# wagnva/semantic-nerf-for-satellite-data

Measured on AMD Instinct MI355X. Metric: train rays/sec (4096 rays x 64 samples), higher is better.
Workload: dtype f32(f16x2)

## Files before the change

### semantic-nerf-for-satellite-data_amd/csrc/api.hip

```cpp
#include <stdarg.h>
#include <stdio.h>
#include <stdlib.h>
#include <string.h>

#include <mutex>

#include "aux_kernels.h"
#include "bsp.h"
#include "composite.h"
#include "gemm.h"
#include "plan.h"

namespace snerf {

int forward_bsp(const Plan& p, const float* pk, const SnerfInputs* in, const SnerfOutputs* out, void* workspace, hipStream_t st);
int backward_bsp(const Plan& p, const float* pk, const SnerfInputs* in, const SnerfOutGrads* go, float* gp, float* d_t, float* d_t_s,
                 void* workspace, hipStream_t st);

static thread_local char g_err[512] = "";
void set_error(const char* fmt, ...) {
  va_list ap;
  va_start(ap, fmt);
  vsnprintf(g_err, sizeof(g_err), fmt, ap);
  va_end(ap);
// ... 195 lines not shown
  size_t off = 0;
  auto take = [&](size_t n) { size_t o = off; off += round_up_sz(n, 64); return o; };
  for (int i = 0; i < p.L; ++i) {
    p.k_tr[i] = (i == 0) ? p.Ep : (((p.skip_mask >> i) & 1u) ? p.Ep + p.W : p.W);
    p.w_tr[i] = take((size_t)p.W * p.k_tr[i]);
    p.b_tr[i] = take(p.W);
  }
  p.w_fs = take((size_t)(p.W + NARROW) * p.W); p.b_fs = take(p.W + NARROW);
  p.w_h1 = take((size_t)p.N1 * p.FA); p.b_h1 = take(p.N1);
  p.w_s2 = take((size_t)p.H * p.H); p.b_s2 = take(p.H);
  p.w_s3 = take((size_t)p.H * p.H); p.b_s3 = take(p.H);
  p.w_s4 = take((size_t)NARROW * p.H); p.b_s4 = take(NARROW);
  p.w_fin = take((size_t)NARROW * p.KF); p.b_fin = take(NARROW);
  p.sky_floats = 9 * p.H + 4;
  p.sky = take(p.sky_floats);
  p.n_fp32 = off;
  {
    const char* ev = getenv("SNERF_COMPOSE_FEATS");
    p.compose_feats = p.pl == 2 && (p.H & 31) == 0 && p.N1 + NARROW <= 2048 && !(ev && ev[0] == '0' && ev[1] == 0);
  }
  if (!p.compose_feats) { plan_weights(p); plan_bsp(p); return SNERF_OK; }
  Plan q = p;
  q.compose_feats = false;
  plan_weights(q);
  plan_bsp(q);
  plan_weights(p);
  plan_bsp(p);
  if (q.packed_floats > p.packed_floats) p.packed_floats = q.packed_floats;
  if (q.ws_bytes > p.ws_bytes) p.ws_bytes = q.ws_bytes;
  return SNERF_OK;
}

struct TableBuilder {
  CopyTable tabs[4];
  int nt = 0;
  bool missing = false;
  TableBuilder() { memset(tabs, 0, sizeof(tabs)); nt = 1; }
  void add(float* user, int user_ld, int rows, int cols, size_t dst_off, int dst_ld) {
    if (!user) { missing = true; return; }
    if (tabs[nt - 1].n == COPY_TABLE_MAX) ++nt;
    CopyEntry& e = tabs[nt - 1].e[tabs[nt - 1].n++];
    e.user = user; e.user_ld = user_ld; e.rows = rows; e.cols = cols; e.dst_off = dst_off; e.dst_ld = dst_ld;
  }
};

static void build_tables(const Plan& p, const SnerfParams* w, TableBuilder& tb) {
// ... 263 lines not shown
```

### semantic-nerf-for-satellite-data_amd/csrc/bsp.h

```cpp
#pragma once
#include "common.h"
#include "gemm.h"

namespace snerf {
namespace bsp {

constexpr int RB = 128;
constexpr int CB = 128;
constexpr int E_MAX = 100;
constexpr int E_QUIET = 60;

typedef __amdgpu_buffer_rsrc_t srd_t;
typedef unsigned int u32x4 __attribute__((ext_vector_type(4)));
typedef unsigned int u32x2 __attribute__((ext_vector_type(2)));
typedef _Float16 f16x8 __attribute__((ext_vector_type(8)));
typedef _Float16 f16x4 __attribute__((ext_vector_type(4)));
constexpr unsigned OOB = 0xFFFFFFF0u;

__host__ __device__ inline int ncb_of(int ld) { return (ld + CB - 1) / CB; }
__host__ __device__ inline size_t plane_bytes(size_t rows, int ld, int pl = 2) { return rows * (size_t)ld * 2 * pl; }
__host__ __device__ inline size_t etab_ints(size_t rows, int ld) { return ((rows + RB - 1) / RB) * (size_t)ncb_of(ld); }
__host__ __device__ inline unsigned g16_off(int k, int pl = 2) { return (unsigned)(k >> 4) * 32u * (unsigned)pl + (unsigned)(k & 15) * 2u; }

__host__ __device__ inline int exp_of_maxbits(unsigned b) {
// ... 55 lines not shown
  const f16x8 h = __builtin_bit_cast(f16x8, hi);
#pragma unroll
  for (int i = 0; i < 8; ++i) x[i] = (float)h[i];
}

__host__ __device__ inline int wf16_row(int m) { return (m & 0x13) | ((m & 4) << 1) | ((m & 8) >> 1); }

struct KcArgs {
  const char* A = nullptr; const int* EA = nullptr; int lda = 0; int a_col0 = 0;
  const char* A2 = nullptr; const int* EA2 = nullptr; int lda2 = 0; int a2_col0 = 0;
  int Ka = 0;
  const char* W = nullptr;
  const int* EW = nullptr;
  int w_rb32 = 0, w_row0 = 0, w_k0 = 0; unsigned w_bytes = 0;
  int I = 0, J = 0, K = 0;
  char* C = nullptr; int* EC = nullptr; int ldc = 0; int c_col0 = 0;
  float* Cf = nullptr;
  const float* bias = nullptr;
  int act = ACT_NONE; float w0 = 1.f;
  unsigned* Csign = nullptr;
  int aux_mode = AUX_NONE;
  const char* H = nullptr; const int* EH = nullptr; int ldh = 0; int h_col0 = 0; const unsigned* Hsign = nullptr;
  float* colsum = nullptr; int ldcs = 0;
  int tiles_i = 0, tiles_j = 0;
  int tj_skip = -1;
  int tiles_jr = 0;
  int rev = 0;
  int dbg = 0;
  int* tile_ctr = nullptr;
  int pl = 2;
  const float* nd_w = nullptr; float* nd_out = nullptr; unsigned long long nd_stride = 0;
  int nd_omax = 0, nd_ldw = 0;
  int nd_rows[8] = {0, 0, 0, 0, 0, 0, 0, 0}, nd_row0[8] = {0, 0, 0, 0, 0, 0, 0, 0}, nd_woff[8] = {0, 0, 0, 0, 0, 0, 0, 0};
};
__host__ __device__ inline size_t sign_words(size_t rows, int ld) { return ((rows + 31) / 32) * (size_t)((ld + 63) / 64) * 64; }

struct DwArgs {
  const char* A = nullptr; const int* EA = nullptr; int lda = 0; int a_col0 = 0;
  const char* B = nullptr; const int* EB = nullptr; int ldb = 0; int b_col0 = 0;
  int I = 0, J = 0, P = 0;
  float* C = nullptr; int ldc = 0;
  int k_split = 0, n_split = 1; unsigned long long slab_stride = 0;
  int tiles_i = 0, tiles_j = 0;
  int pl = 2;
};

// ... 45 lines not shown
constexpr int WPACK_MAX = 48;
struct WPackTable { WPackJob j[WPACK_MAX]; int n; };
constexpr int WPACK_CHUNK = 24;
struct WPackChunk { WPackJob j[WPACK_CHUNK]; int n; };
__host__ __device__ inline size_t wp16_bytes(int rows, int K, int pl = 2) { return (size_t)((rows + 31) / 32) * (size_t)(K / 16) * 1024 * pl; }
int launch_wpack(const WPackTable& tb, const float* master, char* planes, int* exps, unsigned* maxbits, int pl, hipStream_t st);

struct SgJob {
  const float* A = nullptr; long long sa_i = 0, sa_k = 0;
  const float* B = nullptr; long long sb_k = 0, sb_j = 0;
  const float* D = nullptr; int ldd = 0;
  const float* u = nullptr; const float* v = nullptr;
  float* C = nullptr; int ldc = 0;
  int M = 0, N = 0, K = 0, acc = 0;
  int blk0 = 0;
};
constexpr int SG_MAX = 6;
struct SgTable { SgJob j[SG_MAX]; int n = 0; };
int launch_sgemm(const SgTable& tb, int tile_m, hipStream_t st);
void compose_jobs(SgTable& tb, const float* w_h1, const float* w_f, const float* b_f, const float* b_h1, float* wc, float* bc, int W, int FA, int N1);
void uncompose_jobs(SgTable& tb, const float* G, const float* gc, const float* w_h1, const float* w_f, const float* b_f,
                    float* dw_h1, float* db_h1, float* dw_f, float* db_f, int W, int FA, int M);

}
struct EncodeArgs;
namespace bsp {
int launch_encode_bsp(const EncodeArgs& a, char* pe, int* Epe, char* fa, int* Efa, int fa_col0, int pl, hipStream_t st);
int launch_relight_extras(const EncodeArgs& a, char* fa, int* Efa, int fa_col0, int pl, hipStream_t st);
int launch_zero_cols(char* base, size_t pitch, size_t width_bytes, int rows, hipStream_t st);
int launch_colsum32_bsp(const float* in, int rows, float* partial, char* planes, int* E, int pl, hipStream_t st);

}
}
```

### semantic-nerf-for-satellite-data_amd/csrc/bsp_aux.hip

```cpp
#include "bsp.h"
#include "aux_kernels.h"

namespace snerf {
namespace bsp {

__device__ __forceinline__ float block_max_256(float m, float* sm) {
#pragma unroll
  for (int o = 32; o >= 1; o >>= 1) m = fmaxf(m, __shfl_xor(m, o, 64));
  __syncthreads();
  if ((threadIdx.x & 63) == 0) sm[threadIdx.x >> 6] = m;
  __syncthreads();
  return fmaxf(fmaxf(sm[0], sm[1]), fmaxf(sm[2], sm[3]));
}

__global__ __launch_bounds__(256) void to_planes_kernel(const float* __restrict__ src, int ld_src, int rows, int cols,
                                                        char* __restrict__ dst, int* __restrict__ E, int ld, int col0, int pl) {
  __shared__ float sm[4];
  const int rb = blockIdx.y, cb = blockIdx.x;
  const int t = threadIdx.x, c8 = cb * 128 + (t & 15) * 8;
  float v[8][8];
  float m = 0.f;
#pragma unroll
  for (int i = 0; i < 8; ++i) {
    const int r = rb * 128 + (t >> 4) + 16 * i;
// ... 185 lines not shown
  auto job = [&]() -> SgJob& { tb.j[tb.n] = SgJob(); return tb.j[tb.n++]; };
  { SgJob& j = job(); j.A = G; j.sa_i = FA; j.sa_k = 1; j.B = w_f; j.sb_k = 1; j.sb_j = W; j.u = gc; j.v = b_f; j.C = dw_h1; j.ldc = FA; j.M = M; j.N = W; j.K = W; j.acc = 1; }
  { SgJob& j = job(); j.A = w_h1; j.sa_i = 1; j.sa_k = FA; j.B = G; j.sb_k = FA; j.sb_j = 1; j.C = dw_f; j.ldc = W; j.M = W; j.N = W; j.K = M; j.acc = 1; }
  { SgJob& j = job(); j.A = w_h1; j.sa_i = 1; j.sa_k = FA; j.B = gc; j.sb_k = 1; j.sb_j = 0; j.C = db_f; j.ldc = 1; j.M = W; j.N = 1; j.K = M; j.acc = 1; }
  { SgJob& j = job(); j.D = gc; j.ldd = 1; j.C = db_h1; j.ldc = 1; j.M = M; j.N = 1; j.acc = 1; }
}

int launch_sgemm(const SgTable& tb0, int tile_m, hipStream_t st) {
  if (tb0.n <= 0) return SNERF_OK;
  if (tb0.n > SG_MAX || (tile_m != 64 && tile_m != 32)) { set_error("sgemm: bad job table"); return SNERF_ERR_BAD_DESC; }
  SgTable tb = tb0;
  int blocks = 0;
  for (int q = 0; q < tb.n; ++q) {
    SgJob& j = tb.j[q];
    if (!j.C || j.M <= 0 || j.N <= 0 || j.K < 0 || j.ldc < 1 || (j.K > 0 && (!j.A || !j.B)) || (j.u && !j.v) || (j.D && j.ldd < 1)) {
      set_error("sgemm: bad job %d", q);
      return SNERF_ERR_BAD_DESC;
    }
    j.blk0 = blocks;
    blocks += ((j.M + tile_m - 1) / tile_m) * ((j.N + 63) / 64);
  }
  if (tile_m == 64) hipLaunchKernelGGL(sgemm_jobs_kernel<4>, dim3(blocks), dim3(256), 0, st, tb);
  else hipLaunchKernelGGL(sgemm_jobs_kernel<2>, dim3(blocks), dim3(256), 0, st, tb);
  SNERF_LAUNCH_CHECK();
  return SNERF_OK;
}

__global__ void zero_cols_kernel(char* base, size_t pitch, int width16, int rows) {
  const int i = blockIdx.x * blockDim.x + threadIdx.x;
  if (i >= rows * width16) return;
  const int r = i / width16, c = i - r * width16;
  *reinterpret_cast<u32x4*>(base + (size_t)r * pitch + 16 * (size_t)c) = u32x4{0u, 0u, 0u, 0u};
}
int launch_zero_cols(char* base, size_t pitch, size_t width_bytes, int rows, hipStream_t st) {
  const int w16 = (int)(width_bytes / 16);
  if (w16 <= 0 || rows <= 0) return SNERF_OK;
  hipLaunchKernelGGL(zero_cols_kernel, dim3((unsigned)(((size_t)rows * w16 + 255) / 256)), dim3(256), 0, st, base, pitch, w16, rows);
  SNERF_LAUNCH_CHECK();
  return SNERF_OK;
}

__device__ __forceinline__ void point_xyz(const EncodeArgs& a, long long point, float (&x)[3]) {
  const int n = (int)((unsigned)point / (unsigned)a.S);
#pragma unroll
  for (int c = 0; c < 3; ++c) {
    if (a.xyz != nullptr) {
// ... 207 lines not shown
```

### semantic-nerf-for-satellite-data_amd/csrc/bsp_kc.hip

```cpp
#include "bsp_kc_epi.h"

namespace snerf {
namespace bsp {

constexpr int KC_A = 128 * 128, KC_RING = 3;
constexpr int KC_RINGB = KC_RING * KC_A;
constexpr int KC_XREG = KC_RINGB;
constexpr int KC_BIAS = KC_XREG + 4 * 4096;
constexpr int KC_ETAB = KC_BIAS + 2 * 1024;
constexpr int KC_SMAX = KC_ETAB + 2 * 512;
constexpr int KC_NEXT = KC_SMAX + 64;
constexpr int KC_HSIGN = KC_NEXT + 64;
constexpr int KC_LDS = KC_HSIGN + 4 * 1024;
constexpr int KC_NDW = KC_HSIGN;
constexpr int KC_NDW_FLOATS = 2560;
constexpr int KC_LDS_ND = KC_NDW + 4 * KC_NDW_FLOATS;
template <int PL, int ACT, int AUX, bool COLSUM, bool SIGNS, int SINM, bool DIAG = false, int NDOT = 0>
__global__ __launch_bounds__(256, 2) void gemm_kc_kernel(const KcArgs) {
  const kargs_t p = kargs();
  __shared__ __attribute__((aligned(16))) char lds[NDOT > 0 ? KC_LDS_ND : KC_LDS];
  float* smax = reinterpret_cast<float*>(lds + KC_SMAX);
  const int t = threadIdx.x, lane = t & 63;
  const int wave = __builtin_amdgcn_readfirstlane(t >> 6);
  const int wj0 = wave * 64;
  const int tiles_i = p->tiles_i, tiles_j = p->tiles_j, ntiles = tiles_i * tiles_j;
  constexpr int EB = 2 * PL;
  constexpr int KSUB = PL == 2 ? 16 : 32, KSH = PL == 2 ? 4 : 5;
  const int nks16 = p->K >> 4;
  const int nks = (p->K + KSUB - 1) >> KSH;
  const int nks1 = p->Ka < p->K ? p->Ka >> KSH : nks;
  const int eW = *p->EW;
  const int nst = (nks + 1) >> 1, nst1 = nks1 >> 1;
  constexpr bool ONEPASS = ACT == ACT_SIN;
  constexpr bool BIAS = AUX == AUX_NONE && !COLSUM;
  const int dbg = DIAG ? p->dbg : 0;

  auto a_lane_off = [&](int q, int ld, int l) -> unsigned {
    const int row = 8 * (wave + 4 * q) + (l >> 3);
    return (unsigned)row * (unsigned)ld * (unsigned)EB + 16u * (unsigned)((l & 7) ^ ((row >> 1) & 7));
  };
// ... 460 lines not shown
              float sv[8];
              if constexpr (PL == 2) sum8(hh[gg], hl[gg], sv); else cvt8f(hh[gg], sv);
#pragma unroll
              for (int c = 0; c < 8; ++c) {
                const float om = fmaf(-sv[c], sv[c], one_s);
                const float root = __builtin_amdgcn_sqrtf(fabsf(om));
                const unsigned rs = __float_as_uint(root) | ((sword[mi] << (31 - (16 * nj + 8 * gg + c))) & 0x80000000u);
                v[c] *= __uint_as_float(rs);
              }
            } else if (AUX == AUX_RELU_MASK) {
              float hv[8];
              cvt8f(hh[gg], hv);
#pragma unroll
              for (int c = 0; c < 8; ++c) v[c] = hv[c] > 0.f ? v[c] : 0.f;
            }
#pragma unroll
            for (int c = 0; c < 8; ++c) {
              if (COLSUM) cs[8 * gg + c] += v[c];
              acc[mi][nj][8 * gg + c] = v[c];
            }
            if (jw + 16 * gq < e->J) {
              const float m8 = absmax3(v[6], v[7], absmax3(v[4], v[5], absmax3(v[2], v[3], absmax3(v[0], v[1], 0.f))));
              wmax = fmaxf(wmax, (BIAS && (32 * mi + pt) >= nrows) ? 0.f : m8);
            }
          }
        }
        if (COLSUM && e->colsum != nullptr) {
#pragma unroll
          for (int r = 0; r < 16; ++r) cs[r] = sum32(cs[r]);
          if ((el & 31) == 31) {
#pragma unroll
            for (int gg = 0; gg < 2; ++gg)
              if (jw + 16 * (2 * nj + gg) < e->J) {
                float* d = e->colsum + (size_t)c_ti * e->ldcs + jw + 16 * (2 * nj + gg) + 8 * lh;
                *reinterpret_cast<float4*>(d) = make_float4(cs[8 * gg] * fac, cs[8 * gg + 1] * fac, cs[8 * gg + 2] * fac, cs[8 * gg + 3] * fac);
                *reinterpret_cast<float4*>(d + 4) = make_float4(cs[8 * gg + 4] * fac, cs[8 * gg + 5] * fac, cs[8 * gg + 6] * fac, cs[8 * gg + 7] * fac);
              }
          }
        }
      }
      constexpr bool RAW = AUX != AUX_NONE || COLSUM;
      wmax = wave_max(wmax) * (RAW ? fac : 1.f);
      if (el == 0) smax[wave] = wmax;
      barrier_raw();
      const float bmax = fmaxf(smax[wave & 2], smax[(wave & 2) + 1]);
      const int eC = exp_of_maxbits(__float_as_uint(bmax));
// ... 70 lines not shown
  if (a.nd_w != nullptr) {
    if (a.nd_omax == 0) { a.nd_omax = 1; a.nd_ldw = 0; for (int tj = 0; tj < 8; ++tj) { a.nd_rows[tj] = tj < a.tiles_jr ? 1 : 0; a.nd_row0[tj] = 0; } }
    int off = 0;
    for (int tj = 0; tj < a.tiles_jr && tj < 8; ++tj) { a.nd_woff[tj] = off; off += 256 * a.nd_rows[tj]; }
    if (a.tiles_jr > 8 || off > KC_NDW_FLOATS || (a.nd_omax != 1 && a.nd_omax != 5)) { set_error("bsp gemm: folded projections beyond the LDS table"); return SNERF_ERR_BAD_DESC; }
    for (int tj = 0; tj < a.tiles_jr; ++tj) if (a.nd_rows[tj] > a.nd_omax) { set_error("bsp gemm: nd_rows > nd_omax"); return SNERF_ERR_BAD_DESC; }
  }
#ifdef KC_DIAG_BUILD
  constexpr bool DIAG = true;
  static const int dbg = [] { const char* e = getenv("SNERF_KC_DBG"); return e ? atoi(e) : 0; }();
  a.dbg = dbg;
  if (dbg & 2) a.w_bytes = 0;
#else
  constexpr bool DIAG = false;
#endif
  const int ntiles = a.tiles_i * a.tiles_j, slots = kc_slots();
  const dim3 grid(ntiles < slots ? ntiles : slots), block(256);
  const int tok = prof_hook_begin(2.0 * a.I * (double)a.J * a.K, 0, st);
  const bool cs = a.colsum != nullptr;
#define KC_LAUNCH(ACT_, AUX_, CS_, SG_, SM_) do { if (a.pl == 2) hipLaunchKernelGGL((gemm_kc_kernel<2, ACT_, AUX_, CS_, SG_, SM_, DIAG>), grid, block, 0, st, a); \
                                                 else hipLaunchKernelGGL((gemm_kc_kernel<1, ACT_, AUX_, CS_, SG_, SM_, DIAG>), grid, block, 0, st, a); } while (0)
#define KC_LAUNCH_ND(SG_, ND_) do { if (a.pl == 2) hipLaunchKernelGGL((gemm_kc_kernel<2, ACT_SIN, AUX_NONE, false, SG_, SIN_DIRECT, DIAG, ND_>), grid, block, 0, st, a); \
                                    else hipLaunchKernelGGL((gemm_kc_kernel<1, ACT_SIN, AUX_NONE, false, SG_, SIN_DIRECT, DIAG, ND_>), grid, block, 0, st, a); } while (0)
  if (a.aux_mode == AUX_SINREC) KC_LAUNCH(ACT_NONE, AUX_SINREC, true, false, SIN_FRACT);
  else if (a.aux_mode == AUX_RELU_MASK) KC_LAUNCH(ACT_NONE, AUX_RELU_MASK, true, false, SIN_FRACT);
  else if (a.act == ACT_SIN) {
    if (a.nd_w != nullptr && a.nd_omax == 1) { if (a.Csign == nullptr) KC_LAUNCH_ND(false, 1); else KC_LAUNCH_ND(true, 1); }
    else if (a.nd_w != nullptr) { if (a.Csign == nullptr) KC_LAUNCH_ND(false, 5); else KC_LAUNCH_ND(true, 5); }
    else if (a.Csign == nullptr) KC_LAUNCH(ACT_SIN, AUX_NONE, false, false, SIN_DIRECT);
    else KC_LAUNCH(ACT_SIN, AUX_NONE, false, true, SIN_DIRECT);
  }
  else if (a.act == ACT_RELU) KC_LAUNCH(ACT_RELU, AUX_NONE, false, false, SIN_FRACT);
  else if (cs) KC_LAUNCH(ACT_NONE, AUX_NONE, true, false, SIN_FRACT);
  else KC_LAUNCH(ACT_NONE, AUX_NONE, false, false, SIN_FRACT);
#undef KC_LAUNCH
#undef KC_LAUNCH_ND
  SNERF_LAUNCH_CHECK();
  prof_hook_end(tok, st);
  return SNERF_OK;
}

}
}
```

### semantic-nerf-for-satellite-data_amd/csrc/bsp_pass.hip

```cpp
#include "aux_kernels.h"
#include "bsp.h"
#include "composite.h"
#include "plan.h"

namespace snerf {

namespace {
struct Ws {
  char* base;
  char* c(size_t off) const { return base + off; }
  float* f(size_t off) const { return reinterpret_cast<float*>(base + off); }
  int* i(size_t off) const { return reinterpret_cast<int*>(base + off); }
  unsigned* u(size_t off) const { return reinterpret_cast<unsigned*>(base + off); }
  void a(bsp::KcArgs& g, const PlaneT& t, int k, int col0 = 0) const { g.A = c(t.o); g.EA = i(t.e); g.lda = t.ld; g.a_col0 = col0; g.Ka = k; }
  void a2(bsp::KcArgs& g, const PlaneT& t) const { g.A2 = c(t.o); g.EA2 = i(t.e); g.lda2 = t.ld; }
  void out(bsp::KcArgs& g, const PlaneT& t, int col0 = 0) const { g.C = c(t.o); g.EC = i(t.e); g.ldc = t.ld; g.c_col0 = col0; g.Csign = t.s ? u(t.s) : nullptr; }
  void h(bsp::KcArgs& g, const PlaneT& t, int col0 = 0) const { g.H = c(t.o); g.EH = i(t.e); g.ldh = t.ld; g.h_col0 = col0; g.Hsign = t.s ? u(t.s) : nullptr; }
  void dz(bsp::DwArgs& g, const PlaneT& t) const { g.A = c(t.o); g.EA = i(t.e); g.lda = t.ld; g.a_col0 = 0; }
  void x(bsp::DwArgs& g, const PlaneT& t, int col0) const { g.B = c(t.o); g.EB = i(t.e); g.ldb = t.ld; g.b_col0 = col0; }
};
struct WOp { const char* W; const int* EW; int rb32; unsigned bytes; int K; };
WOp wop(const Plan& p, const float* pk, int job) {
  const char* planes = reinterpret_cast<const char*>(pk + p.n_fp32);
  const bsp::WPackJob& w = p.wj.j[job];
// ... 150 lines not shown
  if (p.train) { c.save_T = ws.f(p.o_T); c.save_rgbraw = ws.f(p.o_rgbraw); }
  RC(launch_composite_fwd(c, st));
  return SNERF_OK;
}

namespace {
struct RQ {
  float* base; size_t cap, used = 0; bool over = false;
  RedTable elem, col;
  float* take(size_t floats) {
    const size_t n = round_up_sz(floats, 64);
    if (used + n > cap) { over = true; return base; }
    float* r = base ? base + used : nullptr; used += n; return r;
  }
};
struct DwMat { DwSplit sp; size_t stride; int ldw; float* slab; };
inline int cs_ld(int width) { return (width + 3) & ~3; }

struct BwdRegions {
  float *nar_fin = nullptr, *nar_sun = nullptr, *nar_sig = nullptr;
  DwMat w_fin, w_s4, w_s3, w_s2, w_h1, w_fs;
  float *cs_fin = nullptr, *cs_s3 = nullptr, *cs_s2 = nullptr, *cs_sun = nullptr, *cs_fa = nullptr, *cs_hl = nullptr;
  int ld_cs1 = 0;
  struct Layer { DwMat w, w_gamma; float* cs; } tr[SNERF_MAX_LAYERS];
};
void take_regions(const Plan& p, RQ& rq, BwdRegions& r, bool embed_only = false) {
  auto dw = [&](int rows, int ldw, int cols, bool narrow_rows, int split_rows = 0) {
    DwMat m;
    m.sp = dw_choose_bsp(p.P, split_rows > 0 ? split_rows : rows, cols, narrow_rows);
    m.stride = round_up_sz((size_t)rows * ldw, 64);
    m.ldw = ldw;
    m.slab = rq.take(m.stride * m.sp.ns);
    return m;
  };
  auto cs = [&](int width) { return rq.take((size_t)((p.P + 127) / 128) * cs_ld(width)); };
  auto nar = [&]() { return rq.take((size_t)((p.P + 255) / 256) * NARROW); };
  const int W = p.W, H = p.H;
  if (embed_only) {
    if (p.sc) return;
    r.nar_fin = nar();
    if (p.compose_feats) { r.ld_cs1 = cs_ld(p.h1w); r.cs_fin = cs(p.h1w); }
    else r.cs_fin = cs(p.KF);
    return;
  }
  if (!p.sc) { r.nar_fin = nar(); r.w_fin = dw(NARROW, p.KF, p.KF, true); if (!p.compose_feats) r.cs_fin = cs(p.KF); }
  r.nar_sun = nar(); r.w_s4 = dw(NARROW, H, H, true); r.w_s3 = dw(H, H, H, false); r.w_s2 = dw(H, H, H, false);
  r.cs_s3 = cs(H); r.cs_s2 = cs(H);
  if (p.compose_feats) {
    r.ld_cs1 = cs_ld(p.h1w); r.cs_fin = cs(p.h1w); r.cs_sun = r.cs_fin + (p.sc ? 0 : p.sun_col);
    r.w_h1 = dw(p.h1w, p.FA, p.FA, false);
    r.nar_sig = nar(); r.w_fs = dw(NARROW, W, W, false, W); r.cs_hl = cs(W);
  } else {
    r.cs_sun = cs(H);
    r.w_h1 = dw(p.h1w, p.FA, p.FA, false); r.cs_fa = cs(p.FA);
    r.nar_sig = nar(); r.w_fs = dw(W + NARROW, W, W, false, W); r.cs_hl = cs(W);
  }
  for (int i = p.L - 1; i >= 0; --i) {
    if (i > 0 && ((p.skip_mask >> i) & 1u)) { r.tr[i].w_gamma = dw(W, p.Ep, p.Ep, false); r.tr[i].w = dw(W, W, W, false); }
    else r.tr[i].w = dw(W, p.k_tr[i], i == 0 ? p.Ep : W, false);
    r.tr[i].cs = i > 0 ? cs(W) : nullptr;
  }
}
}

size_t bsp_rq_floats(const Plan& p) {
  RQ rq{nullptr, ~(size_t)0};
  BwdRegions r;
  take_regions(p, rq, r);
  return rq.used;
}

int backward_bsp(const Plan& p, const float* pk, const SnerfInputs* in, const SnerfOutGrads* go, float* gp, float* d_t, float* d_t_s,
                 void* workspace, hipStream_t st) {
  const Ws ws{(char*)workspace};
  const int P = p.P, W = p.W, H = p.H;
  const bool embed = p.embed_grad;
  int kcq = 0;
  auto launch_kc = [&](bsp::KcArgs& g) { g.rev = kcq & 1; g.tile_ctr = kcq < KCQ_SLOTS ? ws.i(p.o_kcq) + 16 * kcq++ : nullptr; return bsp::launch_kc(g, st); };
  RQ rq{ws.f(p.o_rq), p.rq_floats};
  BwdRegions r;
  take_regions(p, rq, r, embed);
  if (rq.over) { set_error("reduction arena too small (plan / pass mismatch)"); return SNERF_ERR_WORKSPACE; }
  auto dact = [&](bsp::KcArgs& g, const PlaneT& h, int col0 = 0, float w0 = 1.f) {
    ws.h(g, h, col0);
    if (p.siren) { g.aux_mode = AUX_SINREC; g.w0 = w0; }
    else g.aux_mode = AUX_RELU_MASK;
  };
  auto colsum = [&](bsp::KcArgs& g, float* cs, int width) { g.colsum = cs; g.ldcs = cs_ld(width); };
  auto bias_from_colsum = [&](const float* cs, int width, float* gout) { return red_add_col(rq.col, cs, (P + 127) / 128, (size_t)cs_ld(width), width, gout); };
  auto dw_gemm = [&](const DwMat& m, const PlaneT& dz, int I, bool narrow_i, const PlaneT& X, int x_col0, int J, size_t slab_off = 0) {
    bsp::DwArgs g;
    ws.dz(g, dz); ws.x(g, X, x_col0);
    g.I = I; g.J = J; g.P = P;
    g.C = m.slab + slab_off; g.ldc = m.ldw;
    g.k_split = m.sp.k_split; g.n_split = m.sp.ns; g.slab_stride = m.stride; g.pl = p.pl;
    return bsp::launch_dw(g, narrow_i, st);
  };
  auto dw_reduce = [&](const DwMat& m, size_t count, float* gout) { return red_add_elem(rq.elem, m.slab, m.sp.ns, m.stride, count, gout); };
  auto narrow_grad = [&](const float* dnar, float* part, const PlaneT& t, float* gout) {
    RC(bsp::launch_colsum32_bsp(dnar, P, part, ws.c(t.o), ws.i(t.e), p.pl, st));
    return red_add_col(rq.col, part, (P + 255) / 256, NARROW, NARROW, gout);
  };
  float* dsig = ws.f(p.o_dsig); float* dfin = ws.f(p.o_dfin); float* dsun = ws.f(p.o_dsun);
  if (embed && p.sc) {
// ... 13 lines not shown
  b.g_beta_s = go->beta_semantic; b.g_logits = go->semantic_logits;
  b.d_sigo = dsig; b.d_fino = dfin; b.d_suno = dsun; b.sky_slab = (p.sc || embed) ? nullptr : ws.f(p.o_skyslab);
  b.zero = ws.u(p.o_kcq); b.zero_n = KCQ_SLOTS * 16;
  RC(launch_composite_bwd(b, st));
  if (!p.sc && !embed)
    RC(red_add_col(rq.col, ws.f(p.o_skyslab), p.comp_blocks * 4, (size_t)p.sky_floats, p.sky_floats, gp + p.sky));


  const PlaneT dz1 = p.dza.view(p.h1w);
  const int sun_col = p.sc ? 0 : p.sun_col;
  if (!p.sc) {
    if (embed) RC(bsp::launch_colsum32_bsp(dfin, P, r.nar_fin, ws.c(p.pdfin.o), ws.i(p.pdfin.e), p.pl, st));
    else {
      RC(narrow_grad(dfin, r.nar_fin, p.pdfin, gp + p.b_fin));
      RC(dw_gemm(r.w_fin, p.pdfin, NARROW, true, p.h1, 0, p.KF));
      RC(dw_reduce(r.w_fin, (size_t)NARROW * p.KF, gp + p.w_fin));
    }
    bsp::KcArgs g;
    ws.a(g, p.pdfin, NARROW); weights(g, p, pk, p.wj_tfin);
    g.I = P; g.J = p.KF; g.K = NARROW; ws.out(g, dz1);
    dact(g, p.h1);
    colsum(g, r.cs_fin, p.KF);
    if (p.compose_feats) g.ldcs = r.ld_cs1;
    RC(launch_kc(g));
    if (!p.compose_feats && !embed) RC(bias_from_colsum(r.cs_fin, p.KF, gp + p.b_h1));
  }
  if (!embed) {
    RC(narrow_grad(dsun, r.nar_sun, p.pdsun, gp + p.b_s4));
    RC(dw_gemm(r.w_s4, p.pdsun, NARROW, true, p.s3, 0, H));
    RC(dw_reduce(r.w_s4, (size_t)NARROW * H, gp + p.w_s4));
    bsp::KcArgs g;
    ws.a(g, p.pdsun, NARROW); weights(g, p, pk, p.wj_ts4);
    g.I = P; g.J = H; g.K = NARROW; ws.out(g, p.dsa);
    dact(g, p.s3);
    colsum(g, r.cs_s3, H);
    RC(launch_kc(g));
    RC(bias_from_colsum(r.cs_s3, H, gp + p.b_s3));
    RC(dw_gemm(r.w_s3, p.dsa, H, false, p.s2, 0, H));
    RC(dw_reduce(r.w_s3, (size_t)H * H, gp + p.w_s3));
    ws.a(g, p.dsa, H); g.K = H; weights(g, p, pk, p.wj_ts3);
    ws.out(g, p.dsb);
    dact(g, p.s2);
    colsum(g, r.cs_s2, H);
    RC(launch_kc(g));
    RC(bias_from_colsum(r.cs_s2, H, gp + p.b_s2));
    RC(dw_gemm(r.w_s2, p.dsb, H, false, p.h1, sun_col, H));
    RC(dw_reduce(r.w_s2, (size_t)H * H, gp + p.w_s2));
    ws.a(g, p.dsb, H); weights(g, p, pk, p.wj_ts2);
    ws.out(g, dz1, sun_col);
    dact(g, p.h1, sun_col);
    colsum(g, r.cs_sun, H);
    if (p.compose_feats) g.ldcs = r.ld_cs1;
    RC(launch_kc(g));
    if (!p.compose_feats) RC(bias_from_colsum(r.cs_sun, H, gp + p.b_h1 + (size_t)p.sun_col));
  }
  auto transient_grads = [&]() {
    const bool want_t = d_t != nullptr, want_ts = d_t_s != nullptr && p.x_ts >= 0;
    if (p.sc) {
      if (want_t) RC(launch_zero_bytes(d_t, (size_t)p.N * p.tau * sizeof(float), st));
      if (want_ts) RC(launch_zero_bytes(d_t_s, (size_t)p.N * p.tau * sizeof(float), st));
    } else if (want_t || want_ts) {
      int b_lo = p.blk_beta, b_hi = p.blk_beta;
      auto use = [&](int blk, bool on) { if (on && blk >= 0) { if (blk < b_lo) b_lo = blk; if (blk > b_hi) b_hi = blk; } };
      use(p.blk_rgb, p.rgb_t); use(p.blk_sem, p.sem_t || p.sem_ts); use(p.blk_sbeta, true);
      const int k_lo = b_lo * H, k_n = (b_hi + 1 - b_lo) * H;
      float* dext = ws.f(p.o_dfin);
      bsp::KcArgs x;
      ws.a(x, dz1, k_n, k_lo); weights(x, p, pk, p.wj_th1, p.Wf, k_lo);
      x.I = P; x.J = p.Xp; x.K = k_n; x.Cf = dext;
      RC(bsp::launch_kc_narrow(x, st));
      if (want_t) RC(launch_ray_sum32(dext, p.x_t, p.N, p.S, p.tau, d_t, st));
      if (want_ts) RC(launch_ray_sum32(dext, p.x_ts, p.N, p.S, p.tau, d_t_s, st));
    }
    return (int)SNERF_OK;
  };
  if (embed) return transient_grads();
  PlaneT dz_cur = p.dza.view(W);
  PlaneT dz_nxt = p.dzb.view(W);
  const bool sig_live = !p.sc || go->weights != nullptr || go->transparency != nullptr || go->sigmas != nullptr;
  const PlaneT& hl = p.h[p.L - 1];
  bool uncompose = false;
  if (p.compose_feats) {
    const int r0 = p.sc ? p.sun_col : 0;
    const int nt = (P + 127) / 128, X = p.FA - W;
    RC(dw_gemm(r.w_h1, dz1, p.h1w, false, p.fa, 0, p.FA));
    RC(red_add_elem2d(rq.elem, r.w_h1.slab + W, r.w_h1.sp.ns, r.w_h1.stride, p.h1w, X, p.FA, gp + p.w_h1 + (size_t)r0 * p.FA + W, p.FA));
    RC(red_add_elem2d(rq.elem, r.w_h1.slab, r.w_h1.sp.ns, r.w_h1.stride, p.h1w, W, p.FA, r.w_h1.slab, p.FA));
    RC(red_store_last(rq.elem));
    RC(red_add_col(rq.col, r.cs_fin, nt, (size_t)r.ld_cs1, p.h1w, r.cs_fin));
    RC(red_store_last(rq.col));
    uncompose = true;
    RC(transient_grads());
    if (sig_live) {
      RC(narrow_grad(dsig, r.nar_sig, p.pdsig, gp + p.b_fs + W));
      RC(dw_gemm(r.w_fs, p.pdsig, NARROW, true, hl, 0, W));
      RC(dw_reduce(r.w_fs, (size_t)NARROW * W, gp + p.w_fs + (size_t)W * W));
    }
    { const PlaneT sw = dz_cur; dz_cur = dz_nxt; dz_nxt = sw; }
    bsp::KcArgs g;
    ws.a(g, dz1, p.h1w);
    if (sig_live) ws.a2(g, p.pdsig);
    weights(g, p, pk, p.wj_th1, 0, r0); g.I = P; g.J = W; g.K = sig_live ? p.h1w + NARROW : p.h1w;
    ws.out(g, dz_cur);
    dact(g, hl, 0, (p.L == 1) ? 30.f : 1.f);
    colsum(g, r.cs_hl, W);
    RC(launch_kc(g));
    RC(bias_from_colsum(r.cs_hl, W, gp + p.b_tr[p.L - 1]));
  }
  const PlaneT dfa = p.dzb.view(p.FA);
  if (!p.compose_feats) {
    const int r0 = p.sc ? p.sun_col : 0;
// ... 29 lines not shown
      RC(dw_gemm(t.w, dz_cur, W, false, p.h[i - 1], 0, W));
      RC(red_add_elem2d(rq.elem, t.w_gamma.slab, t.w_gamma.sp.ns, t.w_gamma.stride, W, p.Ep, p.Ep, gp + p.w_tr[i], p.k_tr[i]));
      RC(red_add_elem2d(rq.elem, t.w.slab, t.w.sp.ns, t.w.stride, W, W, W, gp + p.w_tr[i] + p.Ep, p.k_tr[i]));
    } else {
      if (i == 0) RC(dw_gemm(t.w, dz_cur, W, false, p.pe, 0, p.Ep));
      else RC(dw_gemm(t.w, dz_cur, W, false, p.h[i - 1], 0, W));
      RC(dw_reduce(t.w, (size_t)W * p.k_tr[i], gp + p.w_tr[i]));
    }
    if (i == 0) break;
    bsp::KcArgs g;
    ws.a(g, dz_cur, W); weights(g, p, pk, p.wj_tt[i]);
    g.I = P; g.J = W; g.K = W; ws.out(g, dz_nxt);
    dact(g, p.h[i - 1], 0, (i - 1 == 0) ? 30.f : 1.f);
    colsum(g, t.cs, W);
    RC(launch_kc(g));
    RC(bias_from_colsum(t.cs, W, gp + p.b_tr[i - 1]));
    const PlaneT sw = dz_cur; dz_cur = dz_nxt; dz_nxt = sw;
  }
  RC(launch_reductions(rq.elem, rq.col, st));
  if (!uncompose) return SNERF_OK;
  {
    const size_t r0 = p.sc ? (size_t)p.sun_col : 0;
    bsp::SgTable tb;
    bsp::uncompose_jobs(tb, r.w_h1.slab, r.cs_fin, pk + p.w_h1 + r0 * p.FA, pk + p.w_fs, pk + p.b_fs,
                        gp + p.w_h1 + r0 * p.FA, gp + p.b_h1 + r0, gp + p.w_fs, gp + p.b_fs, W, p.FA, p.h1w);
    return bsp::launch_sgemm(tb, 32, st);
  }
}

}
```

### semantic-nerf-for-satellite-data_amd/csrc/plan.h

```cpp
#pragma once
#include "bsp.h"
#include "common.h"
#include "../../include/snerf_hip.h"

namespace snerf {

constexpr int NARROW = 32;
constexpr int MAX_CLASSES = 16;
constexpr int ND_FIN = 5;
constexpr int MAX_SKY_UNITS = 8;

struct PlaneT { size_t o = 0, e = 0, s = 0; int ld = 0; };
struct PlaneScratch {
  size_t o = 0, e = 0; int maxw = 0;
  PlaneT view(int ld) const { PlaneT t; t.o = o; t.e = e; t.ld = ld; return t; }
};

struct Plan {
  int N = 0, S = 0, P = 0, Pp = 0;
  int W = 0, H = 0, L = 0, E = 0, Ep = 0, F = 0, tau = 0, C = 0;
  bool siren = false, train = false, sc = false, sem_sigmoid = false;
  bool relight = false;
  bool embed_grad = false;
  bool geometry = false;
// ... 21 lines not shown
  size_t packed_floats = 0;
  int pl = 2;

  size_t o_z = 0, o_T = 0, o_rgbraw = 0;
  PlaneT pe, fa, h1, s2, s3, h[SNERF_MAX_LAYERS];
  size_t o_sigo = 0, o_fino = 0, o_suno = 0;
  size_t o_sigpart = 0, o_sunpart = 0, o_finpart = 0;
  bool nd_sig = false, nd_sun = false;
  bool fuse_trunk = false;
  bool nd_fin = false;
  PlaneScratch dza, dzb;
  PlaneT dsa, dsb, pdsig, pdfin, pdsun;
  size_t o_dsig = 0, o_dfin = 0, o_dsun = 0;
  size_t o_skyslab = 0;
  size_t o_kcq = 0;
  size_t o_rq = 0, rq_floats = 0;
  bsp::WPackTable wj = {};
  int wj_tr[SNERF_MAX_LAYERS] = {0}, wj_tt[SNERF_MAX_LAYERS] = {0};
  int wj_fs = 0, wj_sig = 0, wj_tfs = 0, wj_h1 = 0, wj_th1 = 0, wj_s2 = 0, wj_ts2 = 0, wj_s3 = 0, wj_ts3 = 0, wj_s4 = 0, wj_ts4 = 0,
      wj_fin = 0, wj_tfin = 0;
  size_t wp_bytes = 0;
  int h1w = 0;
  bool compose_feats = false;
  int wj_first = 0;
  size_t o_wc = 0;
  size_t o_bc = 0;
  int comp_blocks = 0;
  size_t ws_bytes = 0;
};

inline bool skips_beta_block(const Plan& p, bool want_beta) {
  return p.nd_fin && !p.train && p.H == 256 && p.blk_beta >= 0 && !want_beta && !p.rgb_t && p.blk_sbeta < 0;
}

constexpr int KCQ_SLOTS = 64;
struct DwSplit { int ns = 1; int k_split = 32; };
DwSplit dw_choose_bsp(int P, int rows, int cols, bool narrow_rows);

#define RC(expr) do { int _rc = (expr); if (_rc) return _rc; } while (0)

int make_plan(const SnerfDesc* d, Plan* pl);

size_t bsp_rq_floats(const Plan& p);

}
```

Measured before the change: 169,300.

## Compute per-ray extras weight gradients from per-ray column sums instead of full GEMM

The extras columns of the feature input (transient embeddings etc.) are constant across samples of a ray, so their weight gradient is rewritten as per-ray column sums of the h1 derivative times the 16 per-ray extras. The derivative GEMM now emits per-32-row column sums, which are reduced per ray, and a new kernel forms the outer product and the transient embedding gradients. The big dW GEMM shrinks to the W trunk columns only. This adds extra kernels, reduction arena space and a new code path gated by an environment variable.

```diff
diff --git a/semantic-nerf-for-satellite-data_amd/csrc/api.hip b/semantic-nerf-for-satellite-data_amd/csrc/api.hip
--- a/semantic-nerf-for-satellite-data_amd/csrc/api.hip
+++ b/semantic-nerf-for-satellite-data_amd/csrc/api.hip
@@ -241,6 +241,10 @@
   if (!p.compose_feats) { plan_weights(p); plan_bsp(p); return SNERF_OK; }
   Plan q = p;
   q.compose_feats = false;
+  {
+    const char* ev = getenv("SNERF_RAY_EXTRAS");
+    p.ray_extras = ray_extras_shape(p) && !(ev && ev[0] == '0' && ev[1] == 0);
+  }
   plan_weights(q);
   plan_bsp(q);
   plan_weights(p);
diff --git a/semantic-nerf-for-satellite-data_amd/csrc/bsp.h b/semantic-nerf-for-satellite-data_amd/csrc/bsp.h
--- a/semantic-nerf-for-satellite-data_amd/csrc/bsp.h
+++ b/semantic-nerf-for-satellite-data_amd/csrc/bsp.h
@@ -101,6 +101,7 @@
   int aux_mode = AUX_NONE;
   const char* H = nullptr; const int* EH = nullptr; int ldh = 0; int h_col0 = 0; const unsigned* Hsign = nullptr;
   float* colsum = nullptr; int ldcs = 0;
+  float* colsum32 = nullptr;
   int tiles_i = 0, tiles_j = 0;
   int tj_skip = -1;
   int tiles_jr = 0;
@@ -192,6 +193,16 @@
 void uncompose_jobs(SgTable& tb, const float* G, const float* gc, const float* w_h1, const float* w_f, const float* b_f,
                     float* dw_h1, float* db_h1, float* dw_f, float* db_f, int W, int FA, int M);
 
+struct RayOuterArgs {
+  const float* R = nullptr; long long ldr = 0; int N = 0, M = 0;
+  const float* ext = nullptr;
+  float* dw = nullptr; int lddw = 0;
+  const float* wt = nullptr; int ldw = 0, k0 = 0, kn = 0;
+  float* d_t = nullptr; float* d_ts = nullptr; int x_t = 0, x_ts = -1, tau = 0;
+};
+int launch_ray_outer(const RayOuterArgs& a, hipStream_t st);
+int launch_ext_rows(const char* fa, const int* Efa, int ldfa, int col0, int pl, int N, int S, float* ext, hipStream_t st);
+
 }
 struct EncodeArgs;
 namespace bsp {
diff --git a/semantic-nerf-for-satellite-data_amd/csrc/bsp_aux.hip b/semantic-nerf-for-satellite-data_amd/csrc/bsp_aux.hip
--- a/semantic-nerf-for-satellite-data_amd/csrc/bsp_aux.hip
+++ b/semantic-nerf-for-satellite-data_amd/csrc/bsp_aux.hip
@@ -231,6 +231,108 @@
   }
   if (tile_m == 64) hipLaunchKernelGGL(sgemm_jobs_kernel<4>, dim3(blocks), dim3(256), 0, st, tb);
   else hipLaunchKernelGGL(sgemm_jobs_kernel<2>, dim3(blocks), dim3(256), 0, st, tb);
+  SNERF_LAUNCH_CHECK();
+  return SNERF_OK;
+}
+
+constexpr int RO_RG = 64, RO_JB = 8;
+__global__ __launch_bounds__(RO_JB * RO_RG) void ray_outer_kernel(const RayOuterArgs a) {
+  __shared__ float part[RO_RG][RO_JB][17];
+  const int t = threadIdx.x;
+  const int blocks_dw = a.dw != nullptr ? (a.M + RO_JB - 1) / RO_JB : 0;
+  if ((int)blockIdx.x >= blocks_dw) {
+    const int n = ((int)blockIdx.x - blocks_dw) * (RO_JB * RO_RG / 64) + (t >> 6), l = t & 63;
+    if (n >= a.N) return;
+    float acc[16];
+#pragma unroll
+    for (int c = 0; c < 16; ++c) acc[c] = 0.f;
+    for (int k = l; k < a.kn; k += 64) {
+      const float r = a.R[(size_t)n * a.ldr + a.k0 + k];
+      const float4* w = reinterpret_cast<const float4*>(a.wt + (size_t)(a.k0 + k) * a.ldw);
+#pragma unroll
+      for (int q = 0; q < 4; ++q) {
+        const float4 v = w[q];
+        acc[4 * q] = fmaf(r, v.x, acc[4 * q]); acc[4 * q + 1] = fmaf(r, v.y, acc[4 * q + 1]);
+        acc[4 * q + 2] = fmaf(r, v.z, acc[4 * q + 2]); acc[4 * q + 3] = fmaf(r, v.w, acc[4 * q + 3]);
+      }
+    }
+#pragma unroll
+    for (int c = 0; c < 16; ++c) {
+      float v = acc[c];
+#pragma unroll
+      for (int o = 32; o >= 1; o >>= 1) v += __shfl_xor(v, o, 64);
+      if (l == 0) {
+        if (a.d_t != nullptr && c >= a.x_t && c < a.x_t + a.tau) a.d_t[(size_t)n * a.tau + (c - a.x_t)] = v;
+        if (a.d_ts != nullptr && c >= a.x_ts && c < a.x_ts + a.tau) a.d_ts[(size_t)n * a.tau + (c - a.x_ts)] = v;
+      }
+    }
+    return;
+  }
+  const int jl = t % RO_JB, rg = t / RO_JB;
+  const int j = (int)blockIdx.x * RO_JB + jl;
+  float acc[16];
+#pragma unroll
+  for (int c = 0; c < 16; ++c) acc[c] = 0.f;
+#pragma unroll 4
+  for (int n = rg; n < a.N; n += RO_RG) {
+    const float4* x = reinterpret_cast<const float4*>(a.ext + (size_t)n * 16);
+    const float r = j < a.M ? a.R[(size_t)n * a.ldr + j] : 0.f;
+#pragma unroll
+    for (int q = 0; q < 4; ++q) {
+      const float4 v = x[q];
+      acc[4 * q] = fmaf(r, v.x, acc[4 * q]); acc[4 * q + 1] = fmaf(r, v.y, acc[4 * q + 1]);
+      acc[4 * q + 2] = fmaf(r, v.z, acc[4 * q + 2]); acc[4 * q + 3] = fmaf(r, v.w, acc[4 * q + 3]);
+    }
+  }
+#pragma unroll
+  for (int c = 0; c < 16; ++c) part[rg][jl][c] = acc[c];
+  __syncthreads();
+  if (t < RO_JB * 16) {
+    const int j2 = (int)blockIdx.x * RO_JB + (t >> 4), c = t & 15;
+    float s = 0.f;
+    for (int q = 0; q < RO_RG; ++q) s += part[q][t >> 4][c];
+    if (j2 < a.M) a.dw[(size_t)j2 * a.lddw + c] += s;
+  }
+}
+int launch_ray_outer(const RayOuterArgs& a, hipStream_t st) {
+  if (!a.R || a.N <= 0 || a.M <= 0 || a.ldr < a.M || (a.dw != nullptr && (!a.ext || ((uintptr_t)a.ext & 15) || a.lddw < 16))) {
+    set_error("ray outer: per-ray sums [N][M] and the rays' extras [N][16]");
+    return SNERF_ERR_BAD_DESC;
+  }
+  const bool dt = a.d_t != nullptr || a.d_ts != nullptr;
+  if (dt && (!a.wt || ((uintptr_t)a.wt & 15) || (a.ldw & 3) || a.ldw < 16 || a.k0 < 0 || a.kn <= 0 || a.k0 + a.kn > a.M || a.tau < 1 || a.x_t < 0 || a.x_t + a.tau > 16 ||
+             (a.d_ts != nullptr && (a.x_ts < 0 || a.x_ts + a.tau > 16)))) {
+    set_error("ray outer: d_t from columns [k0, k0 + kn) of the per-ray sums and 16 aligned weight columns");
+    return SNERF_ERR_BAD_DESC;
+  }
+  if (!dt && !a.dw) { set_error("ray outer: nothing to write"); return SNERF_ERR_BAD_DESC; }
+  constexpr int RAYS = RO_JB * RO_RG / 64;
+  const int blocks = (a.dw != nullptr ? (a.M + RO_JB - 1) / RO_JB : 0) + (dt ? (a.N + RAYS - 1) / RAYS : 0);
+  hipLaunchKernelGGL(ray_outer_kernel, dim3((unsigned)blocks), dim3(RO_JB * RO_RG), 0, st, a);
+  SNERF_LAUNCH_CHECK();
+  return SNERF_OK;
+}
+
+__global__ void ext_rows_kernel(const char* __restrict__ fa, const int* __restrict__ Efa, int ldfa, int col0, int pl, int N, int S, float* __restrict__ ext) {
+  const int i = blockIdx.x * blockDim.x + threadIdx.x;
+  if (i >= 2 * N) return;
+  const int n = i >> 1, half = i & 1;
+  const size_t row = (size_t)n * S;
+  const float sc = pow2f(-Efa[(row >> 7) * ncb_of(ldfa) + (col0 >> 7)]);
+  const char* q = fa + row * (size_t)ldfa * 2 * pl + g16_off(col0, pl) + 16 * half;
+  float x[8];
+  const u32x4 hi = *reinterpret_cast<const u32x4*>(q);
+  if (pl == 2) sum8(hi, *reinterpret_cast<const u32x4*>(q + 32), x); else cvt8f(hi, x);
+  float* d = ext + (size_t)n * 16 + 8 * half;
+  *reinterpret_cast<float4*>(d) = make_float4(x[0] * sc, x[1] * sc, x[2] * sc, x[3] * sc);
+  *reinterpret_cast<float4*>(d + 4) = make_float4(x[4] * sc, x[5] * sc, x[6] * sc, x[7] * sc);
+}
+int launch_ext_rows(const char* fa, const int* Efa, int ldfa, int col0, int pl, int N, int S, float* ext, hipStream_t st) {
+  if (!fa || !Efa || !ext || ((uintptr_t)ext & 15) || N <= 0 || S <= 0 || (col0 & 127) || col0 + 16 > ldfa || (pl != 1 && pl != 2)) {
+    set_error("ext rows: an extras block of 16 columns at a multiple of 128 inside the plane tensor");
+    return SNERF_ERR_BAD_DESC;
+  }
+  hipLaunchKernelGGL(ext_rows_kernel, dim3((unsigned)((2 * N + 255) / 256)), dim3(256), 0, st, fa, Efa, ldfa, col0, pl, N, S, ext);
   SNERF_LAUNCH_CHECK();
   return SNERF_OK;
 }
diff --git a/semantic-nerf-for-satellite-data_amd/csrc/bsp_kc.hip b/semantic-nerf-for-satellite-data_amd/csrc/bsp_kc.hip
--- a/semantic-nerf-for-satellite-data_amd/csrc/bsp_kc.hip
+++ b/semantic-nerf-for-satellite-data_amd/csrc/bsp_kc.hip
@@ -15,7 +15,7 @@
 constexpr int KC_NDW = KC_HSIGN;
 constexpr int KC_NDW_FLOATS = 2560;
 constexpr int KC_LDS_ND = KC_NDW + 4 * KC_NDW_FLOATS;
-template <int PL, int ACT, int AUX, bool COLSUM, bool SIGNS, int SINM, bool DIAG = false, int NDOT = 0>
+template <int PL, int ACT, int AUX, bool COLSUM, bool SIGNS, int SINM, bool DIAG = false, int NDOT = 0, bool CSF = false>
 __global__ __launch_bounds__(256, 2) void gemm_kc_kernel(const KcArgs) {
   const kargs_t p = kargs();
   __shared__ __attribute__((aligned(16))) char lds[NDOT > 0 ? KC_LDS_ND : KC_LDS];
@@ -522,6 +522,19 @@
             if (jw + 16 * gq < e->J) {
               const float m8 = absmax3(v[6], v[7], absmax3(v[4], v[5], absmax3(v[2], v[3], absmax3(v[0], v[1], 0.f))));
               wmax = fmaxf(wmax, (BIAS && (32 * mi + pt) >= nrows) ? 0.f : m8);
+            }
+          }
+          if constexpr (COLSUM && CSF) {
+#pragma unroll
+            for (int gg = 0; gg < 2; ++gg) {
+              float f[8];
+#pragma unroll
+              for (int c = 0; c < 8; ++c) f[c] = sum32(acc[mi][nj][8 * gg + c]) * fac;
+              if ((el & 31) == 31 && jw + 16 * (2 * nj + gg) < e->J) {
+                float* d = e->colsum32 + (size_t)(4 * c_ti + mi) * e->ldcs + jw + 16 * (2 * nj + gg) + 8 * lh;
+                *reinterpret_cast<float4*>(d) = make_float4(f[0], f[1], f[2], f[3]);
+                *reinterpret_cast<float4*>(d + 4) = make_float4(f[4], f[5], f[6], f[7]);
+              }
             }
           }
         }
@@ -638,8 +651,10 @@
                                                  else hipLaunchKernelGGL((gemm_kc_kernel<1, ACT_, AUX_, CS_, SG_, SM_, DIAG>), grid, block, 0, st, a); } while (0)
 #define KC_LAUNCH_ND(SG_, ND_) do { if (a.pl == 2) hipLaunchKernelGGL((gemm_kc_kernel<2, ACT_SIN, AUX_NONE, false, SG_, SIN_DIRECT, DIAG, ND_>), grid, block, 0, st, a); \
                                     else hipLaunchKernelGGL((gemm_kc_kernel<1, ACT_SIN, AUX_NONE, false, SG_, SIN_DIRECT, DIAG, ND_>), grid, block, 0, st, a); } while (0)
-  if (a.aux_mode == AUX_SINREC) KC_LAUNCH(ACT_NONE, AUX_SINREC, true, false, SIN_FRACT);
-  else if (a.aux_mode == AUX_RELU_MASK) KC_LAUNCH(ACT_NONE, AUX_RELU_MASK, true, false, SIN_FRACT);
+#define KC_LAUNCH_CSF(AUX_) hipLaunchKernelGGL((gemm_kc_kernel<2, ACT_NONE, AUX_, true, false, SIN_FRACT, DIAG, 0, true>), grid, block, 0, st, a)
+  if (a.colsum32 != nullptr && (a.pl != 2 || a.colsum == nullptr || a.aux_mode == AUX_NONE || ((uintptr_t)a.colsum32 & 15))) { set_error("bsp gemm: per-block column sums need a two-plane derivative launch with colsum"); return SNERF_ERR_BAD_DESC; }
+  if (a.aux_mode == AUX_SINREC) { if (a.colsum32 != nullptr) KC_LAUNCH_CSF(AUX_SINREC); else KC_LAUNCH(ACT_NONE, AUX_SINREC, true, false, SIN_FRACT); }
+  else if (a.aux_mode == AUX_RELU_MASK) { if (a.colsum32 != nullptr) KC_LAUNCH_CSF(AUX_RELU_MASK); else KC_LAUNCH(ACT_NONE, AUX_RELU_MASK, true, false, SIN_FRACT); }
   else if (a.act == ACT_SIN) {
     if (a.nd_w != nullptr && a.nd_omax == 1) { if (a.Csign == nullptr) KC_LAUNCH_ND(false, 1); else KC_LAUNCH_ND(true, 1); }
     else if (a.nd_w != nullptr) { if (a.Csign == nullptr) KC_LAUNCH_ND(false, 5); else KC_LAUNCH_ND(true, 5); }
@@ -650,6 +665,7 @@
   else if (cs) KC_LAUNCH(ACT_NONE, AUX_NONE, true, false, SIN_FRACT);
   else KC_LAUNCH(ACT_NONE, AUX_NONE, false, false, SIN_FRACT);
 #undef KC_LAUNCH
+#undef KC_LAUNCH_CSF
 #undef KC_LAUNCH_ND
   SNERF_LAUNCH_CHECK();
   prof_hook_end(tok, st);
diff --git a/semantic-nerf-for-satellite-data_amd/csrc/bsp_pass.hip b/semantic-nerf-for-satellite-data_amd/csrc/bsp_pass.hip
--- a/semantic-nerf-for-satellite-data_amd/csrc/bsp_pass.hip
+++ b/semantic-nerf-for-satellite-data_amd/csrc/bsp_pass.hip
@@ -196,9 +196,11 @@
   DwMat w_fin, w_s4, w_s3, w_s2, w_h1, w_fs;
   float *cs_fin = nullptr, *cs_s3 = nullptr, *cs_s2 = nullptr, *cs_sun = nullptr, *cs_fa = nullptr, *cs_hl = nullptr;
   int ld_cs1 = 0;
+  float* cs_blk = nullptr; int ld_R = 0;
+  float* ext32 = nullptr;
   struct Layer { DwMat w, w_gamma; float* cs; } tr[SNERF_MAX_LAYERS];
 };
-void take_regions(const Plan& p, RQ& rq, BwdRegions& r, bool embed_only = false) {
+void take_regions(const Plan& p, RQ& rq, BwdRegions& r, bool ray_extras, bool embed_only = false) {
   auto dw = [&](int rows, int ldw, int cols, bool narrow_rows, int split_rows = 0) {
     DwMat m;
     m.sp = dw_choose_bsp(p.P, split_rows > 0 ? split_rows : rows, cols, narrow_rows);
@@ -215,6 +217,7 @@
     r.nar_fin = nar();
     if (p.compose_feats) { r.ld_cs1 = cs_ld(p.h1w); r.cs_fin = cs(p.h1w); }
     else r.cs_fin = cs(p.KF);
+    if (ray_extras) { r.cs_blk = rq.take((size_t)((p.P + 127) / 128) * 4 * r.ld_cs1); r.ld_R = (p.S / 32) * r.ld_cs1; }
     return;
   }
   if (!p.sc) { r.nar_fin = nar(); r.w_fin = dw(NARROW, p.KF, p.KF, true); if (!p.compose_feats) r.cs_fin = cs(p.KF); }
@@ -222,7 +225,10 @@
   r.cs_s3 = cs(H); r.cs_s2 = cs(H);
   if (p.compose_feats) {
     r.ld_cs1 = cs_ld(p.h1w); r.cs_fin = cs(p.h1w); r.cs_sun = r.cs_fin + (p.sc ? 0 : p.sun_col);
-    r.w_h1 = dw(p.h1w, p.FA, p.FA, false);
+    if (ray_extras) {
+      r.cs_blk = rq.take((size_t)((p.P + 127) / 128) * 4 * r.ld_cs1); r.ld_R = (p.S / 32) * r.ld_cs1; r.ext32 = rq.take((size_t)p.N * 16);
+      r.w_h1 = dw(p.h1w, p.FA, W, false);
+    } else r.w_h1 = dw(p.h1w, p.FA, p.FA, false);
     r.nar_sig = nar(); r.w_fs = dw(NARROW, W, W, false, W); r.cs_hl = cs(W);
   } else {
     r.cs_sun = cs(H);
@@ -238,10 +244,14 @@
 }
 
 size_t bsp_rq_floats(const Plan& p) {
-  RQ rq{nullptr, ~(size_t)0};
-  BwdRegions r;
-  take_regions(p, rq, r);
-  return rq.used;
+  size_t n = 0;
+  for (int rx = 0; rx <= (ray_extras_shape(p) ? 1 : 0); ++rx) {
+    RQ rq{nullptr, ~(size_t)0};
+    BwdRegions r;
+    take_regions(p, rq, r, rx != 0);
+    if (rq.used > n) n = rq.used;
+  }
+  return n;
 }
 
 int backward_bsp(const Plan& p, const float* pk, const SnerfInputs* in, const SnerfOutGrads* go, float* gp, float* d_t, float* d_t_s,
@@ -253,7 +263,8 @@
   auto launch_kc = [&](bsp::KcArgs& g) { g.rev = kcq & 1; g.tile_ctr = kcq < KCQ_SLOTS ? ws.i(p.o_kcq) + 16 * kcq++ : nullptr; return bsp::launch_kc(g, st); };
   RQ rq{ws.f(p.o_rq), p.rq_floats};
   BwdRegions r;
-  take_regions(p, rq, r, embed);
+  const bool rx = p.ray_extras;
+  take_regions(p, rq, r, rx, embed);
   if (rq.over) { set_error("reduction arena too small (plan / pass mismatch)"); return SNERF_ERR_WORKSPACE; }
   auto dact = [&](bsp::KcArgs& g, const PlaneT& h, int col0 = 0, float w0 = 1.f) {
     ws.h(g, h, col0);
@@ -313,6 +324,7 @@
     dact(g, p.h1);
     colsum(g, r.cs_fin, p.KF);
     if (p.compose_feats) g.ldcs = r.ld_cs1;
+    if (rx) g.colsum32 = r.cs_blk + (g.colsum - r.cs_fin);
     RC(launch_kc(g));
     if (!p.compose_feats && !embed) RC(bias_from_colsum(r.cs_fin, p.KF, gp + p.b_h1));
   }
@@ -342,6 +354,7 @@
     dact(g, p.h1, sun_col);
     colsum(g, r.cs_sun, H);
     if (p.compose_feats) g.ldcs = r.ld_cs1;
+    if (rx) g.colsum32 = r.cs_blk + (g.colsum - r.cs_fin);
     RC(launch_kc(g));
     if (!p.compose_feats) RC(bias_from_colsum(r.cs_sun, H, gp + p.b_h1 + (size_t)p.sun_col));
   }
@@ -350,7 +363,7 @@
     if (p.sc) {
       if (want_t) RC(launch_zero_bytes(d_t, (size_t)p.N * p.tau * sizeof(float), st));
       if (want_ts) RC(launch_zero_bytes(d_t_s, (size_t)p.N * p.tau * sizeof(float), st));
-    } else if (want_t || want_ts) {
+    } else if (!rx && (want_t || want_ts)) {
       int b_lo = p.blk_beta, b_hi = p.blk_beta;
       auto use = [&](int blk, bool on) { if (on && blk >= 0) { if (blk < b_lo) b_lo = blk; if (blk > b_hi) b_hi = blk; } };
       use(p.blk_rgb, p.rgb_t); use(p.blk_sem, p.sem_t || p.sem_ts); use(p.blk_sbeta, true);
@@ -365,7 +378,31 @@
     }
     return (int)SNERF_OK;
   };
-  if (embed) return transient_grads();
+  auto ray_sums = [&](int cols) {
+    if (p.S == 32) return 0;
+    RC(red_add_elem2d(rq.elem, r.cs_blk, p.S / 32, (size_t)r.ld_cs1, p.N, cols, r.ld_R, r.cs_blk, r.ld_R));
+    return red_store_last(rq.elem);
+  };
+  auto ray_outer = [&](float* dw) {
+    bsp::RayOuterArgs o;
+    o.R = r.cs_blk; o.ldr = r.ld_R; o.N = p.N; o.M = p.h1w;
+    o.dw = dw; o.lddw = p.FA;
+    if (dw != nullptr) { o.ext = r.ext32; RC(bsp::launch_ext_rows(ws.c(p.fa.o), ws.i(p.fa.e), p.fa.ld, p.Wf, p.pl, p.N, p.S, r.ext32, st)); }
+    if (!p.sc && (d_t != nullptr || (d_t_s != nullptr && p.x_ts >= 0))) {
+      int b_lo = p.blk_beta, b_hi = p.blk_beta;
+      auto use = [&](int blk, bool on) { if (on && blk >= 0) { if (blk < b_lo) b_lo = blk; if (blk > b_hi) b_hi = blk; } };
+      use(p.blk_rgb, p.rgb_t); use(p.blk_sem, p.sem_t || p.sem_ts); use(p.blk_sbeta, true);
+      o.wt = pk + p.w_h1 + p.Wf; o.ldw = p.FA; o.k0 = b_lo * H; o.kn = (b_hi + 1 - b_lo) * H;
+      o.d_t = d_t; o.d_ts = p.x_ts >= 0 ? d_t_s : nullptr; o.x_t = p.x_t; o.x_ts = p.x_ts; o.tau = p.tau;
+    } else if (dw == nullptr) return (int)SNERF_OK;
+    return bsp::launch_ray_outer(o, st);
+  };
+  if (embed) {
+    if (!rx) return transient_grads();
+    RC(ray_sums(p.KF));
+    RC(launch_reductions(rq.elem, rq.col, st));
+    return ray_outer(nullptr);
+  }
   PlaneT dz_cur = p.dza.view(W);
   PlaneT dz_nxt = p.dzb.view(W);
   const bool sig_live = !p.sc || go->weights != nullptr || go->transparency != nullptr || go->sigmas != nullptr;
@@ -374,10 +411,11 @@
   if (p.compose_feats) {
     const int r0 = p.sc ? p.sun_col : 0;
     const int nt = (P + 127) / 128, X = p.FA - W;
-    RC(dw_gemm(r.w_h1, dz1, p.h1w, false, p.fa, 0, p.FA));
-    RC(red_add_elem2d(rq.elem, r.w_h1.slab + W, r.w_h1.sp.ns, r.w_h1.stride, p.h1w, X, p.FA, gp + p.w_h1 + (size_t)r0 * p.FA + W, p.FA));
+    RC(dw_gemm(r.w_h1, dz1, p.h1w, false, p.fa, 0, rx ? W : p.FA));
+    if (!rx) RC(red_add_elem2d(rq.elem, r.w_h1.slab + W, r.w_h1.sp.ns, r.w_h1.stride, p.h1w, X, p.FA, gp + p.w_h1 + (size_t)r0 * p.FA + W, p.FA));
     RC(red_add_elem2d(rq.elem, r.w_h1.slab, r.w_h1.sp.ns, r.w_h1.stride, p.h1w, W, p.FA, r.w_h1.slab, p.FA));
     RC(red_store_last(rq.elem));
+    if (rx) RC(ray_sums(p.h1w));
     RC(red_add_col(rq.col, r.cs_fin, nt, (size_t)r.ld_cs1, p.h1w, r.cs_fin));
     RC(red_store_last(rq.col));
     uncompose = true;
@@ -453,6 +491,7 @@
   {
     const size_t r0 = p.sc ? (size_t)p.sun_col : 0;
     bsp::SgTable tb;
+    if (rx) RC(ray_outer(gp + p.w_h1 + r0 * p.FA + p.Wf));
     bsp::uncompose_jobs(tb, r.w_h1.slab, r.cs_fin, pk + p.w_h1 + r0 * p.FA, pk + p.w_fs, pk + p.b_fs,
                         gp + p.w_h1 + r0 * p.FA, gp + p.b_h1 + r0, gp + p.w_fs, gp + p.b_fs, W, p.FA, p.h1w);
     return bsp::launch_sgemm(tb, 32, st);
diff --git a/semantic-nerf-for-satellite-data_amd/csrc/plan.h b/semantic-nerf-for-satellite-data_amd/csrc/plan.h
--- a/semantic-nerf-for-satellite-data_amd/csrc/plan.h
+++ b/semantic-nerf-for-satellite-data_amd/csrc/plan.h
@@ -67,6 +67,7 @@
   size_t wp_bytes = 0;
   int h1w = 0;
   bool compose_feats = false;
+  bool ray_extras = false;
   int wj_first = 0;
   size_t o_wc = 0;
   size_t o_bc = 0;
@@ -77,6 +78,8 @@
 inline bool skips_beta_block(const Plan& p, bool want_beta) {
   return p.nd_fin && !p.train && p.H == 256 && p.blk_beta >= 0 && !want_beta && !p.rgb_t && p.blk_sbeta < 0;
 }
+
+inline bool ray_extras_shape(const Plan& p) { return p.compose_feats && p.train && p.S % 32 == 0; }
 
 constexpr int KCQ_SLOTS = 64;
 struct DwSplit { int ns = 1; int k_split = 32; };
```

Result: no change. 170,600 (median of 6 runs) (+0.8%).
